# bytedance/DeepSolid

Hardware: AMD Instinct MI355X
Metric: local-energy evals/sec (higher is better)
Workload: dtype f64; 1 GPU; bcc_li 24 e- (12,12), total_energy primal (E_kin forward-Laplacian + Ewald), default detnet ((256,32),)*3, 8 dets; batch_per_gpu=4096, global_batch=4096, parallelism=walker-dp1

## Files before the change

### deepsolid_amd/_lib.py

```python
import ctypes as C
import os

_HERE = os.path.dirname(os.path.abspath(__file__))
LIB_PATH = os.environ.get('DEEPSOLID_HIP_LIB') or os.path.join(_HERE, 'libdeepsolid_hip.so')

DS_MAX_LAYERS = 8
DS_MAX_SYM = 6
_PD = C.POINTER(C.c_double)


class SystemDesc(C.Structure):
    _fields_ = [
        ('dtype', C.c_int32), ('n_up', C.c_int32), ('n_dn', C.c_int32), ('n_atoms_prim', C.c_int32),
        ('prim_atoms', _PD), ('prim_a', C.c_double * 9), ('sim_a', C.c_double * 9), ('n_sym', C.c_int32),
        ('prim_AV', C.c_double * (DS_MAX_SYM * 3)), ('prim_BV', C.c_double * (DS_MAX_SYM * 3)),
        ('sim_AV', C.c_double * (DS_MAX_SYM * 3)), ('sim_BV', C.c_double * (DS_MAX_SYM * 3)),
        ('n_layers', C.c_int32), ('hidden_single', C.c_int32 * DS_MAX_LAYERS),
        ('hidden_double', C.c_int32 * DS_MAX_LAYERS), ('n_det', C.c_int32), ('distance_type', C.c_int32),
        ('envelope_type', C.c_int32), ('full_det', C.c_int32), ('use_last_layer', C.c_int32),
        ('bias_orbitals', C.c_int32), ('klist_up', _PD), ('klist_dn', _PD),
        ('n_atoms_sim', C.c_int32), ('sim_atoms', _PD), ('sim_charges', _PD), ('dist_mode', C.c_int32),
        ('n_g', C.c_int32), ('gpoints', _PD), ('gweight', _PD), ('ion_exp_re', _PD), ('ion_exp_im', _PD),
        ('ewald_alpha', C.c_double), ('ee_const', C.c_double), ('ei_const', C.c_double), ('ii_total', C.c_double),
    ]


class ParamBlock(C.Structure):
    _fields_ = [('offset', C.c_int64), ('rows', C.c_int32), ('cols', C.c_int32)]


class KfacBlock(C.Structure):
    _fields_ = [('kind', C.c_int32), ('index', C.c_int32), ('n_param_blocks', C.c_int32), ('param_blocks', C.c_int32 * 3),
                ('has_bias', C.c_int32), ('d_in', C.c_int32), ('d_out', C.c_int32), ('repeats', C.c_int32),
                ('a_offset', C.c_int64), ('g_offset', C.c_int64)]


_VP = C.c_void_p
SIGNATURES = {
    'ds_device_widths': (C.c_int, [C.POINTER(C.c_int32), C.POINTER(C.c_int32), C.c_int32, C.c_int32, C.c_int32, C.c_int32,
                                   C.POINTER(C.c_int32), C.POINTER(C.c_int32), C.POINTER(C.c_int32), C.POINTER(C.c_int32)]),
    'ds_system_create': (C.c_int, [C.POINTER(SystemDesc), C.POINTER(_VP)]),
    'ds_system_destroy': (None, [_VP]),
    'ds_last_error': (C.c_char_p, []),
    'ds_param_count': (C.c_int64, [_VP]),
    'ds_int8_layers': (C.c_int, [_VP]),
    'ds_param_layout': (C.c_int, [_VP, C.POINTER(ParamBlock), C.c_int]),
    'ds_workspace_bytes': (C.c_int64, [_VP, C.c_int64]),
    'ds_logpsi': (C.c_int, [_VP, _VP, _VP, C.c_int64, _VP, _VP, _VP, C.c_int64, _VP]),
    'ds_logpsi_grad': (C.c_int, [_VP, _VP, _VP, C.c_int64, _VP, _VP, _VP, _VP, C.c_int64, _VP]),
    'ds_vjp_workspace_bytes': (C.c_int64, [_VP, C.c_int64]),
    'ds_logpsi_vjp': (C.c_int, [_VP, _VP, _VP, C.c_int64, _VP, _VP, _VP, _VP, _VP, C.c_int64, _VP]),
    'ds_pretrain_workspace_bytes': (C.c_int64, [_VP, C.c_int64]),
    'ds_pretrain_loss_vjp': (C.c_int, [_VP, _VP, _VP, C.c_int64, _VP, _VP, _VP, _VP, _VP, C.c_int64, _VP]),
    'ds_kfac_block_count': (C.c_int, [_VP]),
    'ds_kfac_layout': (C.c_int, [_VP, C.POINTER(KfacBlock), C.c_int]),
    'ds_kfac_workspace_bytes': (C.c_int64, [_VP, C.c_int64]),
    'ds_kfac_factors': (C.c_int, [_VP, _VP, _VP, C.c_int64, _VP, _VP, _VP, C.c_int64, _VP]),
    'ds_orbitals': (C.c_int, [_VP, _VP, _VP, C.c_int64, _VP, _VP, _VP, C.c_int64, _VP]),
    'ds_ewald': (C.c_int, [_VP, _VP, C.c_int64, _VP, _VP]),
    'ds_local_energy': (C.c_int, [_VP, _VP, _VP, C.c_int64, _VP, _VP, _VP, _VP, _VP, C.c_int64, _VP]),
    'ds_enforce_pbc': (C.c_int, [_PD, C.c_int, _VP, C.c_int64, _VP, _VP, _VP]),
    'ds_observables_workspace_bytes': (C.c_int64, [C.c_int64, C.c_int]),
    'ds_observables': (C.c_int, [_PD, C.c_int, _VP, C.c_int64, C.c_int64, C.POINTER(C.c_int32), C.c_int, C.c_int, _VP, _VP,
                                 C.c_int64, _VP]),
    'ds_mh_propose': (C.c_int, [_VP, _VP, _VP, C.c_double, C.c_int64, _VP, _VP]),
    'ds_mh_accept': (C.c_int, [_VP, _VP, _VP, _VP, _VP, _VP, C.c_int64, _VP, _VP]),
    'ds_mh_propose_ex': (C.c_int, [_VP, C.c_int, _VP, _VP, C.c_double, _VP, C.c_int, C.c_int64, _VP, _VP, _VP]),
    'ds_mh_accept_ex': (C.c_int, [_VP, C.c_int, _VP, _VP, _VP, _VP, _VP, _VP, C.c_double, _VP, _VP, C.c_int, C.c_int64, _VP, _VP, _VP]),
    'ds_mcmc_workspace_bytes': (C.c_int64, [_VP, C.c_int64]),
    'ds_mcmc_step': (C.c_int, [_VP, _VP, _VP, _VP, C.c_int64, C.c_int, C.c_double, C.c_uint64, C.c_uint64, _VP, _VP, C.c_int, _VP, _VP,
                              C.c_int64, _VP]),
    'ds_mcmc_step_one_electron': (C.c_int, [_VP, _VP, _VP, _VP, C.c_int64, C.c_int, C.c_int, C.c_double, C.c_uint64, C.c_uint64, _VP, _VP,
                                           C.c_int, _VP, _VP, C.c_int64, _VP]),
    'ds_mcmc_step_importance': (C.c_int, [_VP, _VP, _VP, _VP, C.c_int64, C.c_int, C.c_double, C.c_uint64, C.c_uint64, _VP, _VP, C.c_int,
                                         _VP, _VP, C.c_int64, _VP]),
    'ds_mcmc_step_asymmetric': (C.c_int, [_VP, _VP, _VP, _VP, C.c_int64, C.c_int, C.c_double, _VP, C.c_int, C.c_uint64, C.c_uint64, _VP, _VP,
                                         C.c_int, _VP, _VP, C.c_int64, _VP]),
    'ds_philox_host': (None, [C.c_uint64, C.c_uint64, C.c_uint64, C.c_uint64, C.c_int, C.POINTER(C.c_uint32)]),
# ... 38 lines not shown
```

### deepsolid_amd/csrc/ds_api.hip

```cpp
#include <hip/hip_runtime.h>

#include <algorithm>
#include <cmath>
#include <cstdarg>
#include <cstdio>
#include <cstdlib>
#include <cstring>
#include <string>
#include <vector>

#include "../../include/deepsolid_hip.h"
#include "ds_grad.h"
#include "ds_kfac.h"
#include "ds_tiles.h"
#include "ds_mcmc.h"
#include "ds_obs.h"
#include "ds_i8.h"

namespace ds {
#define DS_DECL(p) const TileOps<double>* tile_ops_f64_p##p(int); const TileOps<float>* tile_ops_f32_p##p(int);
DS_DECL(0) DS_DECL(1) DS_DECL(2) DS_DECL(3) DS_DECL(4)
#undef DS_DECL
template <> const TileOps<double>* tile_ops<double>(int st) {
    const TileOps<double>* (*parts[])(int) = {tile_ops_f64_p0, tile_ops_f64_p1, tile_ops_f64_p2, tile_ops_f64_p3, tile_ops_f64_p4};
// ... 359 lines not shown
    HIP_OK(hipMemcpyAsync(dr->out, src, m * sizeof(T), hipMemcpyDeviceToDevice, st));
    dr->written = (int64_t)m;
    return 0;
}

inline bool i8_shape(const ds_system* s, int l) {
    const ds::SysDev<double>& S = s->sd;
    return s->dtype == 0 && l >= 1 && s->res1[l] && S.h1[l + 1] == ds::i8::NOUT && S.h1[l] + S.nch * S.h2[l] == 320;
}
inline bool int8_value_layer(const ds_system* s, int l) { return s->use_i8_val && ds::PV == ds::i8::P && i8_shape(s, l); }

inline void i8_prepare(ds_system* s, int l, const double* Wloc, int Kloc, int Nout, hipStream_t st, uint8_t** wp, double** sw) {
    const size_t slot = ds::i8::wp_bytes(64 * 5) + ds::i8::NOUT * sizeof(double);
    *wp = (uint8_t*)s->i8_wp + (size_t)l * slot;
    *sw = (double*)(*wp + ds::i8::wp_bytes(64 * 5));
    if (s->i8_prepped[l] != s->call_seq) {
        hipLaunchKernelGGL(ds::i8::k_i8_prep_w, dim3(ds::i8::NOUT / 16), dim3(256), 0, st, Wloc, Kloc, Nout, *wp, *sw);
        s->i8_prepped[l] = s->call_seq;
    }
}

enum class LayerKind {
    Dense,
    DenseRes,
    L0Stats,
    L0Epi9Means,
    LowRank1,
    Int8
};
struct PairPlan {
    bool res, res_sep;
    bool expand;
    bool write_out;
    unsigned xz; int EW, NW; size_t xlds;
};
struct LayerPlan {
    LayerKind kind;
    bool res_sep;
    bool wide;
    bool pm_mask;
    bool pm_unwritten;
    int prof_kind;
    PairPlan pair;
};
enum class OrbKind { Orb3, Wide, Ldsb, Gemm };
template <typename T> struct ChainPlan {
    const ds::TileOps<T>* to;
    bool lr_on;
    int lr_nc;
    int g4;
    LayerPlan layer[DS_MAX_LAYERS];
    OrbKind orb[2];
    int count(LayerKind k, int n_layers) const {
        int n = 0;
        for (int l = 0; l < n_layers; ++l) n += layer[l].kind == k ? 1 : 0;
        return n;
    }
};

template <typename T>
int plan_chain(const ds_system* s, bool dump, ChainPlan<T>* p) {
    const ds::SysDev<double>& S = s->sd;
    const ds::TileOps<T>* to = p->to = ds::tile_ops<T>(S.P / 16);
    if (!to) return fail("no kernel instance for %d slot tiles (N = %d electrons)", S.P / 16, S.N);
    const int ST = to->ST;
    const bool wide = s->use_wide && to->gemm_wide != nullptr;
    auto gemm_wide = [&](int epi) { return wide && (s->wide_all || ds::gemm_wide_faster<T>(epi)); };
    const int K0loc = S.h1[0] + S.nch * S.h2[0], K0sh = S.nch * S.h1[0];
    p->lr_nc = std::max(2, (K0loc + K0sh + 4 + 15) / 16);
    p->lr_on = !dump && s->use_lr && S.n_layers >= 2 && !s->res1[0] && p->lr_nc <= 4 && S.h1[1] % 16 == 0 && (S.nch * S.h2[1]) % 4 == 0 &&
               3 * (K0loc + K0sh + 4) <= S.h1[1] && p->lr_nc * S.h1[1] < (S.h1[1] - K0loc - K0sh - 4) * ST;
    const int used = S.D - 16 * (ST - 1);
    p->g4 = !s->use_g4 ? 0 : (ST == 5 && used > 8 && used <= 12) ? 3 : (ST == 10 && used <= 4) ? 1 : 0;
    for (int l = 0; l < S.n_layers; ++l) {
        const int Kh = S.h1[l], K2 = S.h2[l], Nout = S.h1[l + 1], Kloc = Kh + S.nch * K2;
        LayerPlan& lp = p->layer[l];
        lp = LayerPlan{};
        if (Nout % 64 || Nout > 1024) return fail("hidden_single must be a multiple of 64 and <= 1024 (got %d)", Nout);
        if (l < S.n_double) {
            PairPlan& pp = lp.pair;
            const int K2o = S.h2[l + 1];
            if (K2o != 32 && K2o != 16) return fail("hidden_double must be 16 or 32 (got %d)", K2o);
            if (K2 % 4) return fail("pair-stream width %d is not a multiple of 4", K2);
            pp.res_sep = s->res2[l] && l == 0;
            pp.res = s->res2[l] && !pp.res_sep;
            pp.xz = (!pp.res && K2o == 32) ? 2 : 1;
            pp.write_out = l + 1 < S.n_double || s->use_last;
            pp.EW = (pp.write_out && S.N % 16 == 8 && pp.xz == 2) ? 2 : 1;
            pp.NW = (pp.EW * S.N + 15) / 16;
            pp.xlds = ((size_t)(K2o / pp.xz) * 5 * pp.EW * S.N + (size_t)pp.EW * S.nch * (K2o / pp.xz) * 5) * sizeof(T);
            pp.expand = !dump && s->use_pair_expand && !pp.res_sep && l + 1 < S.n_layers && pp.NW <= 8 && pp.xlds <= 150 * 1024;
        }
        const bool res = s->res1[l];
        lp.res_sep = res && l == 0 && (Kloc % 16 != 0 || S.nf * S.A != Nout);
        if (res && !lp.res_sep && Kloc % 16) return fail("residual layer with K = %d: the GEMM's operand ring needs K %% 16 == 0", Kloc);
        if (p->lr_on && l == 1) {
            lp.kind = LayerKind::LowRank1;
            lp.wide = wide && (s->wide_all || ds::lr_wide_faster<T>(p->lr_nc));
        } else if (p->lr_on && l == 0) {
            const bool one_kernel = to->layer0_stats && ds::layer0_stats_instance(ST, K0loc / 4);
            lp.kind = one_kernel ? LayerKind::L0Stats : LayerKind::L0Epi9Means;
            lp.wide = !one_kernel && gemm_wide(9);
        } else if (s->use_i8 && S.P == ds::i8::P && i8_shape(s, l)) {
            lp.kind = LayerKind::Int8;
        } else if (res && !lp.res_sep) {
            lp.kind = LayerKind::DenseRes;
            lp.wide = gemm_wide(2);
        } else {
            lp.kind = LayerKind::Dense;
            lp.wide = gemm_wide(1);
        }
        lp.prof_kind = l == 0 ? DS_PROF_SINGLE_FIRST : (lp.kind == LayerKind::LowRank1 ? DS_PROF_SINGLE_LR : DS_PROF_SINGLE_HIDDEN);
        lp.pm_mask = s->use_pm_skip && (l == 0 || (lp.kind == LayerKind::DenseRes && Kh % 16 == 0 && K2 % 16 == 0));
        lp.pm_unwritten = !dump && l >= 1 && !lp.wide &&
                          (lp.kind == LayerKind::LowRank1 ? s->use_pm_skip : (lp.pm_mask && ds::pm_instance<T>(ST)));
    }
    const int Korb = S.h1[S.n_layers] + (s->use_last ? S.nch * S.h2[S.n_layers] : 0);
    if (Korb % 16) return fail("orbital head with K = %d: the GEMM's operand ring needs K %% 16 == 0", Korb);
    for (int sp = 0; sp < S.nch; ++sp) {
        const int OC = S.ocols[sp];
        if (to->gemm_orb3 && OC % 256 != 0 && OC % 192 == 0) p->orb[sp] = OrbKind::Orb3;
        else if (gemm_wide(5)) p->orb[sp] = OrbKind::Wide;
        else if (to->orbital_lb && s->use_ldsb && OC % 64 == 0) p->orb[sp] = OrbKind::Ldsb;
        else p->orb[sp] = OrbKind::Gemm;
// ... 80 lines not shown
    const bool lr_on = plan.lr_on;
    const int K0loc = S.h1[0] + S.nch * S.h2[0], K0sh = S.nch * S.h1[0];
    {
        ProfScope ps(s, DS_PROF_FEATURES, st);
        size_t sh = (size_t)(9 * S.N) * sizeof(T) + (size_t)S.N * S.A * S.nf * sizeof(ds::Jet5<T>);
        hipLaunchKernelGGL((ds::k_features<T>), dim3((unsigned)Bc), dim3(256), sh, st, S, x, blk(s->i_pi[0]), blk(s->i_sg[0]),
                           blk(s->i_pi[S.nch - 1]), blk(s->i_sg[S.nch - 1]), lr_on ? c.XL : c.G[0], lr_on ? K0loc : S.ldk, c.MEAN[0], c.H2[0], c.Q);
    }
    if (lr_on) {
        const int n = S.h1[1] * 16 * lr_nc;
        hipLaunchKernelGGL((ds::k_lr_w0t<T>), dim3((unsigned)((n + 255) / 256)), dim3(256), 0, st, blk(s->i_wloc[0]), blk(s->i_wsh[0]), K0loc, K0sh,
                           S.h1[1], 16 * lr_nc, (T*)s->lr_w0t);
    }
    if (stop == STOP_MEAN0) return copy_out(dr, c.MEAN[0], (size_t)S.nch * S.h1[0] * S.P * Bc, st);
    if (stop == STOP_H2_0) return copy_out(dr, c.H2[0], (size_t)S.h2[0] * 5 * S.NP * Bc, st);
    if (stop == STOP_Q) return copy_out(dr, c.Q, L.Q * Bc, st);
    int gi = 0, hi = 0;
    for (int l = 0; l < S.n_layers; ++l) {
        const LayerPlan& lp = plan.layer[l];
        const int Kh = S.h1[l], K2 = S.h2[l], Nout = S.h1[l + 1];
        if (!(l > 0 && plan.layer[l - 1].pair.expand)) {
            ProfScope ps(s, DS_PROF_M2_EXPAND, st);
            const bool xl = lr_on && l == 0;
            hipLaunchKernelGGL((ds::k_m2_expand<T>), dim3(S.N, (unsigned)Bc, m2_split<T>(K2, S.N)), dim3(256), (size_t)(K2 * 5 * S.N + S.nch * K2 * 5) / m2_split<T>(K2, S.N) * sizeof(T), st, S,
                               c.H2[hi], K2, xl ? c.XL : c.G[gi], Kh, xl ? K0loc : S.ldk, lp.pm_unwritten ? 1 : 0);
        }
        if (stop == STOP_G0 + l) return copy_out(dr, c.G[gi], L.G * Bc, st);
        if (l < S.n_double) {
            const PairPlan& pp = lp.pair;
            const int K2o = S.h2[l + 1];
            const T* W2 = blk(s->i_w2[l]); const T* b2 = blk(s->i_b2[l]);
            ProfScope ps(s, DS_PROF_TWO_LAYER, st);
            if (pp.expand) {
#define DS_TWOX(NT2, RES) hipLaunchKernelGGL((ds::k_two_layer_expand<T, NT2, RES>), dim3(S.N / pp.EW, (unsigned)Bc, pp.xz), dim3(64 * pp.NW), pp.xlds, st, S, c.H2[hi], K2, W2, b2, \
                                             pp.write_out ? c.H2[hi ^ 1] : (T*)nullptr, c.G[gi ^ 1], S.h1[l + 1], S.ldk, plan.layer[l + 1].pm_unwritten ? 1 : 0, pp.EW)
                if (K2o == 32 && pp.res) DS_TWOX(2, true);
                else if (pp.res) DS_TWOX(1, true);
                else DS_TWOX(1, false);
#undef DS_TWOX
            } else {
                const dim3 grid((S.NP / 16 + 3) / 4, (unsigned)Bc);
#define DS_TWO(NT2, RES) hipLaunchKernelGGL((ds::k_two_layer<T, NT2, RES, false>), grid, dim3(256), 0, st, S, c.H2[hi], K2, W2, b2, c.H2[hi ^ 1])
                if (K2o == 32) { if (pp.res) DS_TWO(2, true); else DS_TWO(2, false); }
                else { if (pp.res) DS_TWO(1, true); else DS_TWO(1, false); }
#undef DS_TWO
            }
            if (pp.res_sep)
                hipLaunchKernelGGL((ds::k_pair_res_add<T>), dim3((unsigned)(((size_t)K2o * 5 * S.NP + 255) / 256), (unsigned)Bc), dim3(256), 0, st, c.H2[hi], K2, c.H2[hi ^ 1], K2o,
                                   S.nf, S.NP);
        }
        const int Kloc = Kh + S.nch * K2, Ksh = S.nch * Kh;
        {
            dim3 block; unsigned gz;
            gemm_geom(Nout, NB, &block, &gz, ST);
            dim3 wblock; unsigned wgz;
            gemm_geom(Nout, 4, &wblock, &wgz, 6);
            const size_t gws = (size_t)S.N * S.ldk * S.P, gts = (size_t)S.ldk * S.P;
            const bool lr1 = lp.kind == LayerKind::LowRank1;
            T* Sl = lr1 ? c.ZB + (size_t)Bc * S.h1[1] * S.P : c.ZB;
            {
                ProfScope ps(s, DS_PROF_SHARED_TERM, st);
                if (l == 0 || lr1) {
                    const ds::GemmArgs<T> ga{nullptr, 0, 0, nullptr, 0, l == 0 ? c.MEAN[0] : c.MEAN[1], (size_t)Ksh * S.P, blk(s->i_wsh[l]), Ksh, 0,
                                             Sl, (size_t)Nout * S.P, 0, Nout, S.P, nullptr, blk(s->i_b[l]), ds::OrbEpi<T>{}};
                    to->gemm(6, dim3(1, (unsigned)Bc, gz), block, st, ga);
                } else {
                    dim3 sblock; unsigned sgz;
                    gemm_geom(Nout, NB, &sblock, &sgz);
                    if (ST > 10 && sblock.x > 512) { sblock = dim3(512); sgz = (unsigned)((Nout / (16 * NB) + 7) / 8); }
                    to->shared_term(dim3(1, (unsigned)Bc, sgz), sblock, 2 * 16 * S.P * sizeof(T), st, S, c.G[gi], blk(s->i_wsh[l]), Kh, Sl, Nout, S.P,
                                    blk(s->i_b[l]), 0);
                }
// ... 23 lines not shown
            case LayerKind::L0Epi9Means: {
                ga.Z = c.YO; ga.zws = L.YO; ga.zts = (size_t)2 * Nout;
                layer_gemm(9, ga);
                constexpr int STC = 5;
                const unsigned nfb = (unsigned)((Nout + 63) / 64), nck = (unsigned)((S.P / 16 + STC - 1) / STC);
                hipLaunchKernelGGL((ds::k_layer0_means<T, STC>), dim3(S.nch * nfb * nck, (unsigned)Bc), dim3(256), 0, st, S, c.XL,
                                   (size_t)S.N * K0loc * S.P, (size_t)K0loc * S.P, blk(s->i_wloc[0]), K0loc, c.ZB, Nout, S.P, c.YO, c.MEAN[1]);
                break;
            }
            case LayerKind::Int8: {
                uint8_t* wp; double* sw;
                i8_prepare(s, l, (const double*)blk(s->i_wloc[l]), Kloc, Nout, st, &wp, &sw);
                const int ntiles = (int)(Bc * S.N);
                const dim3 igrid((unsigned)std::min<int64_t>(ntiles, s->n_cu));
                hipLaunchKernelGGL((ds::i8::k_layer_i8<5, 2>), igrid, dim3(512), ds::i8::lds_bytes(), st, (const double*)c.G[gi], gts, (const uint4*)wp,
                                   (const double*)sw, (const double*)Sl, S.N, (double*)c.G[gi ^ 1], ntiles);
                break;
            }
            case LayerKind::DenseRes:
                ga.oe.dbg = s->dbg & 3;
                ga.oe.g4 = plan.g4;
                if (l > 0 && s->prof_on && (s->prof_only < 0 || s->prof_only == DS_PROF_SINGLE_HIDDEN)) { ga.oe.clk = s->clk_dev; ga.oe.dbg = s->dbg; }
                layer_gemm(2, ga);
                break;
            case LayerKind::Dense:
                layer_gemm(1, ga);
                if (lp.res_sep)
                    hipLaunchKernelGGL((ds::k_layer_res_add<T>), dim3(S.N, (unsigned)Bc), dim3(256), 0, st, Xin, xws, xts, c.G[gi ^ 1], gws, gts, S.nf * S.A, Nout, S.P);
                break;
            }
        }
        gi ^= 1;
        if (l < S.n_double) {
            hi ^= 1;
            if (stop == STOP_H2_1 + l) return copy_out(dr, c.H2[hi], (size_t)S.h2[l + 1] * 5 * S.NP * Bc, st);
        }
    }
    if (stop == STOP_G0 + S.n_layers) return copy_out(dr, c.G[gi], L.G * Bc, st);
    const int Kl = S.h1[S.n_layers], K2l = S.h2[S.n_layers];
    if (s->use_last) {
        ProfScope ps(s, DS_PROF_M2_EXPAND, st);
        hipLaunchKernelGGL((ds::k_m2_expand<T>), dim3(S.N, (unsigned)Bc, m2_split<T>(K2l, S.N)), dim3(256), (size_t)(K2l * 5 * S.N + S.nch * K2l * 5) / m2_split<T>(K2l, S.N) * sizeof(T), st, S,
                           c.H2[hi], K2l, c.G[gi], Kl, S.ldk, 0);
    }
    for (int sp = 0; sp < S.nch; ++sp) {
        const int ns = sp == 0 ? S.n_up : S.n_dn, i0 = sp == 0 ? 0 : S.n_up, OC = S.ocols[sp];
        const int Korb = Kl + (s->use_last ? S.nch * K2l : 0);
        dim3 block; unsigned gz;
        gemm_geom(OC, NB, &block, &gz, ST);
        if (s->use_last) {
            ProfScope ps(s, DS_PROF_SHARED_TERM, st);
            to->shared_term(dim3(1, (unsigned)Bc, gz), block, 2 * 16 * S.P * sizeof(T), st, S, c.G[gi], blk(s->i_wsh_orb[sp]), Kl, c.ZB, OC, S.P,
                            (const T*)nullptr, 0);
        }
        ProfScope ps(s, DS_PROF_ORBITAL, st);
        const int ch = S.mat_ch[sp];
        ds::OrbEpi<T> oe{c.Q, c.MOUT, L.MOUT, L.mout_off[ch], S.N, i0, S.nparam[sp], S.nparam_max, S.norb[sp], S.det_n[ch],
                         S.row_off[sp], S.bias_orb ? blk(s->i_borb[sp]) : (const T*)nullptr, nullptr};
        oe.g4 = plan.g4;
        const ds::GemmArgs<T> ga{c.G[gi] + (size_t)i0 * S.ldk * S.P, (size_t)S.N * S.ldk * S.P, (size_t)S.ldk * S.P, blk(s->i_worb[sp]), Korb,
                                 nullptr, 0, nullptr, 0, ns, nullptr, 0, 0, OC, S.P, s->use_last ? (const T*)c.ZB : (const T*)nullptr, nullptr, oe};
        dim3 ob; unsigned oz;
        switch (plan.orb[sp]) {
        case OrbKind::Orb3:
            gemm_geom(OC, 3, &ob, &oz);
            to->gemm_orb3(dim3(ns * oz, (unsigned)Bc, 1), ob, st, ga);
            break;
// ... 1124 lines not shown
    s->wide_all = getenv("DS_WIDE_ALL") != nullptr;
    {
        ChainPlan<double> plan;
        bool need = plan_chain<double>(s, true, &plan) == 0 && plan.count(LayerKind::Int8, s->sd.n_layers) > 0;
        for (int l = 1; l < s->sd.n_layers; ++l) need = need || int8_value_layer(s, l);
        if (need && hipMalloc(&s->i8_wp, (size_t)DS_MAX_LAYERS * (ds::i8::wp_bytes(64 * 5) + ds::i8::NOUT * sizeof(double))) != hipSuccess) {
            ds_system_destroy(s);
            return fail("hipMalloc of the int8 layer's weight planes failed");
        }
    }
    if (const char* e = getenv("DS_CHUNK_WALKERS")) s->chunk_cap = std::min<int64_t>(65535, std::max<int64_t>(1, atol(e)));
    *out = s;
    return 0;
}

void ds_system_destroy(ds_system* s) {
    if (!s) return;
    if (s->clk_dev) (void)hipFree(s->clk_dev);
    if (s->lr_w0t) (void)hipFree(s->lr_w0t);
    if (s->i8_wp) (void)hipFree(s->i8_wp);
    if (s->blob64) (void)hipFree(s->blob64);
    if (s->blob32) (void)hipFree(s->blob32);
    delete s;
}

int64_t ds_param_count(const ds_system* s) { return s ? s->nparams : -1; }

int ds_int8_layers(const ds_system* s) {
    if (!s) return -1;
    ChainPlan<double> plan;
    return plan_chain<double>(s, false, &plan) == 0 ? plan.count(LayerKind::Int8, s->sd.n_layers) : 0;
}

int ds_param_layout(const ds_system* s, ds_param_block* blocks, int max_blocks) {
    if (!s) return -1;
    const int n = (int)s->blocks.size();
    for (int i = 0; i < n && i < max_blocks; ++i) blocks[i] = s->blocks[i];
    return n;
}

int64_t ds_workspace_bytes(const ds_system* s, int64_t B) {
    if (!s) return -1;
    const int64_t esz = s->dtype == 0 ? 8 : 4;
    int64_t budget = (int64_t)80 << 30;
    size_t free_b = 0, total_b = 0;
    if (hipMemGetInfo(&free_b, &total_b) == hipSuccess && free_b > 0)
        budget = std::min<int64_t>(budget, std::max<int64_t>((int64_t)(free_b / 10 * 4), (int64_t)1 << 30));
    const int64_t cap = s->chunk_cap;
    int64_t chunk = std::min<int64_t>(std::max<int64_t>(B, 1), cap);
    chunk = std::max<int64_t>(1, std::min<int64_t>(chunk, budget / ((int64_t)s->ws.per_walker * esz)));
    int64_t groups = std::min<int64_t>((std::max<int64_t>(B, 1) + ds::PV - 1) / ds::PV, 64);
    groups = std::max<int64_t>(1, std::min<int64_t>(groups, budget / ((int64_t)s->wsv.per_walker * esz)));
    return std::max((int64_t)s->ws.per_walker * esz * chunk, (int64_t)s->wsv.per_walker * esz * groups) + 256;
}

int ds_local_energy(ds_system* s, const void* params, const void* x, int64_t B, void* out_ke, void* out_ewald, void* out_logabs,
                    void* out_phase, void* ws, int64_t ws_bytes, void* stream) {
    if (s) ++s->call_seq;
    if (!s || !params || !x || !ws) return fail("null argument");
    if (B <= 0) return 0;
    hipStream_t st = (hipStream_t)stream;
    return s->dtype == 0 ? local_energy_impl<double>(s, params, x, B, out_ke, out_ewald, out_logabs, out_phase, ws, ws_bytes, st)
                         : local_energy_impl<float>(s, params, x, B, out_ke, out_ewald, out_logabs, out_phase, ws, ws_bytes, st);
}

int ds_logpsi(ds_system* s, const void* params, const void* x, int64_t B, void* out_logabs, void* out_phase, void* ws,
// ... 455 lines not shown
```

### deepsolid_amd/csrc/ds_kernels.h

```cpp
#pragma once
#include "ds_device.h"

namespace ds {

#define DS_MAXL 8

template <typename T> struct SysDev {
    int N, n_up, n_dn, A, L, K, nch;
    int D, P, NP;
    int n_layers, n_double;
    int h1[DS_MAXL + 1];
    int h2[DS_MAXL + 1];
    int ldk;
    int full_det, env_type, bias_orb;
    int dist_type, nf;
    int norb[2];
    int n_detch;
    int det_n[2];
    int mat_ch[2], row_off[2];
    int nparam[2];
    int nparam_max;
    int ocols[2];
    const T *prim_a, *prim_ainv, *sim_a, *sim_ainv, *prim_AV, *prim_BV, *sim_AV, *sim_BV, *atoms;
    const T* klist[2];
// ... 269 lines not shown
        pm_last = pm_valid && (lr == 15 || seg_of(p + 1) != sg);
    }
#pragma unroll
    for (int a = 0; a < NT2; ++a)
#pragma unroll
        for (int r = 0; r < 4; ++r) {
            const int n = 16 * a + acc_row<T>(lane, r);
            const T z0 = acc[a][0][r] + bias[n];
            const T y = ds_tanh(z0), d1 = 1 - y * y, d2 = -2 * y * d1;
            const T z1 = acc[a][1][r], z2 = acc[a][2][r], z3 = acc[a][3][r], z4 = acc[a][4][r];
            T o[5] = {y, d1 * z1, d1 * z2, d1 * z3, d1 * z4 + d2 * 2 * (z1 * z1 + z2 * z2 + z3 * z3)};
            if (VAL) {
                o[1] = ds_tanh(z1 + bias[n]); o[2] = ds_tanh(z2 + bias[n]); o[3] = ds_tanh(z3 + bias[n]); o[4] = ds_tanh(z4 + bias[n]);
            }
#pragma unroll
            for (int c = 0; c < 5; ++c) {
                T v = o[c];
                if (RES) v = ((KEEP ? bk[KEEP ? 4 * a + r : 0][c] : Hw[(size_t)(n * 5 + c) * NP]) + v) * rs2;
                if (Hout) Ho[(size_t)(n * 5 + c) * NP] = v;
                if (VAL && PARTM) {
                    const T pre = row16_prefix(pm_valid ? v : T(0));
                    if (pm_last) pm_lds[(pm_slot * Kout + n) * 5 + c] = pre;
                }
            }
        }
    if (VAL && PARTM) {
        __builtin_amdgcn_fence(__ATOMIC_ACQ_REL, "wavefront");
        __builtin_amdgcn_wave_barrier();
        T* pm = PARTM + ((size_t)w * (NP / 16) + pt) * (PM_SLOTS * Kout * 5);
        for (int i = lane; i < PM_SLOTS * Kout * 5; i += 64) pm[i] = pm_lds[i];
    }
}

template <typename T, int NT2, bool RES>
__global__ void __launch_bounds__(512) k_two_layer_expand(SysDev<T> S, const T* __restrict__ Hin, int Kin, const T* __restrict__ W,
                                                          const T* __restrict__ bias, T* __restrict__ Hout, T* __restrict__ G, int row0,
                                                          int ldg, int skip, int EW) {
    typedef typename Acc4<T>::type acc_t;
    extern __shared__ __attribute__((aligned(16))) char smem_raw[];
    const int w = blockIdx.y, wave = threadIdx.x >> 6, lane = threadIdx.x & 63, tid = threadIdx.x, nt = blockDim.x;
    const int N = S.N, NP = S.NP, P = S.P, Kout = 16 * NT2, e0 = blockIdx.x * EW, PW = EW * N;
    const int KT = Kout * gridDim.z, n0 = Kout * blockIdx.z;
    const int lr = lane & 15, lq = lane >> 4;
    const bool valid = wave * 16 + lr < PW;
    const int pl = valid ? wave * 16 + lr : PW - 1;
    const T* Hw = Hin + (size_t)w * Kin * 5 * NP + e0 * N + pl;
    T* hs = reinterpret_cast<T*>(smem_raw);
    T* sums = hs + Kout * 5 * PW;
    acc_t acc[NT2][5];
#pragma unroll
    for (int a = 0; a < NT2; ++a)
#pragma unroll
        for (int c = 0; c < 5; ++c) acc[a][c] = acc_t{0, 0, 0, 0};
    constexpr bool KEEP = RES && sizeof(T) == 8;
    T bk[KEEP ? 4 * NT2 : 1][5];
    if constexpr (KEEP) {
#pragma unroll
        for (int ks = 0; ks < 4 * NT2; ++ks)
#pragma unroll
            for (int c = 0; c < 5; ++c) bk[ks][c] = Hw[(size_t)((4 * ks + lq) * 5 + c) * NP];
#pragma unroll
        for (int ks = 0; ks < 4 * NT2; ++ks) {
            T av[NT2];
#pragma unroll
            for (int a = 0; a < NT2; ++a) av[a] = W[(size_t)(4 * ks + lq) * KT + n0 + 16 * a + lr];
#pragma unroll
            for (int a = 0; a < NT2; ++a)
#pragma unroll
                for (int c = 0; c < 5; ++c) acc[a][c] = mfma16(av[a], bk[ks][c], acc[a][c]);
        }
    } else
    for (int ks = 0; ks < Kin / 4; ++ks) {
        T av[NT2], bv[5];
#pragma unroll
        for (int a = 0; a < NT2; ++a) av[a] = W[(size_t)(4 * ks + lq) * KT + n0 + 16 * a + lr];
#pragma unroll
        for (int c = 0; c < 5; ++c) bv[c] = Hw[(size_t)((4 * ks + lq) * 5 + c) * NP];
#pragma unroll
        for (int a = 0; a < NT2; ++a)
#pragma unroll
            for (int c = 0; c < 5; ++c) acc[a][c] = mfma16(av[a], bv[c], acc[a][c]);
    }
    const T rs2 = T(0.70710678118654752440);
    T* Ho = (Hout && valid) ? Hout + ((size_t)w * KT + n0) * 5 * NP + e0 * N + pl : nullptr;
#pragma unroll
    for (int a = 0; a < NT2; ++a)
#pragma unroll
        for (int r = 0; r < 4; ++r) {
            const int n = 16 * a + acc_row<T>(lane, r);
            const T z0 = acc[a][0][r] + bias[n0 + n];
            const T y = ds_tanh(z0), d1 = 1 - y * y, d2 = -2 * y * d1;
            const T z1 = acc[a][1][r], z2 = acc[a][2][r], z3 = acc[a][3][r], z4 = acc[a][4][r];
            const T o[5] = {y, d1 * z1, d1 * z2, d1 * z3, d1 * z4 + d2 * 2 * (z1 * z1 + z2 * z2 + z3 * z3)};
// ... 1017 lines not shown
```

### deepsolid_amd/device.py

```python
import ctypes as C

import numpy as np
import torch

from . import _lib

_DTYPES = {torch.float64: 0, torch.float32: 1}


def _pd(a):
    return a.ctypes.data_as(C.POINTER(C.c_double))


def _ptr(t):
    return C.c_void_p(t.data_ptr()) if t is not None else C.c_void_p(0)


def _stream():
    return C.c_void_p(torch.cuda.current_stream().cuda_stream)


def _require_gpu():
    if not torch.cuda.is_available():
        raise RuntimeError('deepsolid_amd needs a ROCm GPU: there is no CPU path (the CPU oracle lives in '
# ... 551 lines not shown
                self._ws.numel(), _stream()), 'ds_mcmc_step_importance')
            return n_accept
        if first_electron is not None:
            _lib.check(self.lib.ds_mcmc_step_one_electron(
                self.handle, _ptr(p), _ptr(x), _ptr(lp), B, int(steps), int(first_electron), float(width), int(seed) & (2 ** 64 - 1),
                int(offset) & (2 ** 64 - 1), _ptr(normals), _ptr(uniforms), int(bool(lp_valid)), _ptr(n_accept), _ptr(self._ws),
                self._ws.numel(), _stream()), 'ds_mcmc_step_one_electron')
            return n_accept
        _lib.check(self.lib.ds_mcmc_step(self.handle, _ptr(p), _ptr(x), _ptr(lp), B, int(steps), float(width),
                                         int(seed) & (2 ** 64 - 1), int(offset) & (2 ** 64 - 1), _ptr(normals), _ptr(uniforms),
                                         int(bool(lp_valid)), _ptr(n_accept), _ptr(self._ws), self._ws.numel(), _stream()),
                   'ds_mcmc_step')
        return n_accept

    def energy_stats(self, ke, ew):
        out = torch.empty(8, dtype=torch.float64, device=self.device)
        _lib.check(self.lib.ds_energy_stats(self.handle, _ptr(ke), _ptr(ew), ke.shape[0], _ptr(out), _stream()), 'ds_energy_stats')
        return out

    def profile(self, on=True, only=None):
        mode = 0 if not on else (1 if only is None else 2 + _lib.PROF_KINDS.index(only))
        _lib.check(self.lib.ds_profile_enable(self.handle, mode), 'ds_profile_enable')

    def profile_read(self):
        n = len(_lib.PROF_KINDS)
        ms = (C.c_double * n)()
        cnt = (C.c_int64 * n)()
        _lib.check(self.lib.ds_profile_read(self.handle, ms, cnt), 'ds_profile_read')
        return {k: (float(ms[i]), int(cnt[i])) for i, k in enumerate(_lib.PROF_KINDS)}

    def int8_layers(self):
        return int(self.lib.ds_int8_layers(self.handle))

    def profile_clock(self):
        cyc, ticks = C.c_double(0), C.c_double(0)
        _lib.check(self.lib.ds_profile_read_clock(self.handle, C.byref(cyc), C.byref(ticks)), 'ds_profile_read_clock')
        return cyc.value, ticks.value, (cyc.value / ticks.value * 0.1 if ticks.value > 0 else None)

    def debug_stage(self, params, x, stage, n_elems):
        x = self._check_x(x)
        p = self.pack_params(params)
        ws = self.workspace(x.shape[0])
        out = torch.zeros(int(n_elems), dtype=self.dtype, device=self.device)
        n = self.lib.ds_debug_stage(self.handle, _ptr(p), _ptr(x), x.shape[0], stage.encode(), _ptr(out), out.numel(),
                                    _ptr(ws), ws.numel(), _stream())
        if n < 0:
            raise RuntimeError(f'ds_debug_stage({stage}): {self.lib.ds_last_error().decode()}')
        return out[:n]


def observable_sums(recvec, x, q_int, pol_direction):
    _require_gpu()
    if not x.is_cuda:
        raise RuntimeError('observable_sums: walkers must live on the ROCm device (no CPU path)')
    if x.dtype not in _DTYPES:
        raise TypeError(f'observable_sums: walkers must be float64 or float32, got {x.dtype}')
    if x.dim() != 2 or x.shape[1] % 3:
        raise ValueError(f'observable_sums: walkers must have shape (B, 3N), got {tuple(x.shape)}')
    if x.shape[0] < 1:
        raise ValueError('observable_sums: empty walker batch (the observables are batch means)')
    lib = _lib.load()
    x = x.contiguous()
    rv = np.ascontiguousarray(np.asarray(recvec, dtype=np.float64).reshape(3, 3))
    q = np.ascontiguousarray(np.asarray(q_int, dtype=np.int32).reshape(-1, 3))
    B, n_q = x.shape[0], q.shape[0]
    need = lib.ds_observables_workspace_bytes(B, n_q)
# ... 7 lines not shown
```

### include/deepsolid_hip.h

```cpp
#ifndef DEEPSOLID_HIP_H
#define DEEPSOLID_HIP_H

#include <stddef.h>
#include <stdint.h>

#ifdef __cplusplus
extern "C" {
#endif

#define DS_MAX_LAYERS 8
#define DS_MAX_SYM 6

typedef struct ds_system ds_system;

typedef struct ds_system_desc {
    int32_t dtype;
    int32_t n_up, n_dn;
    int32_t n_atoms_prim;
    const double* prim_atoms;
    double prim_a[9];
    double sim_a[9];
    int32_t n_sym;
    double prim_AV[DS_MAX_SYM * 3], prim_BV[DS_MAX_SYM * 3];
    double sim_AV[DS_MAX_SYM * 3], sim_BV[DS_MAX_SYM * 3];
// ... 7 lines not shown
    int32_t use_last_layer;
    int32_t bias_orbitals;
    const double* klist_up;
    const double* klist_dn;
    int32_t n_atoms_sim;
    const double* sim_atoms;
    const double* sim_charges;
    int32_t dist_mode;
    int32_t n_g;
    const double* gpoints;
    const double* gweight;
    const double* ion_exp_re;
    const double* ion_exp_im;
    double ewald_alpha;
    double ee_const;
    double ei_const;
    double ii_total;
} ds_system_desc;

typedef struct ds_param_block {
    int64_t offset;
    int32_t rows, cols;
} ds_param_block;

int ds_device_widths(const int32_t* hidden_single, const int32_t* hidden_double, int32_t n_layers, int32_t n_in_single,
                     int32_t n_in_double, int32_t n_double, int32_t* dev_single, int32_t* dev_double, int32_t* res_single,
                     int32_t* res_double);

int ds_system_create(const ds_system_desc* desc, ds_system** out);
void ds_system_destroy(ds_system* sys);
const char* ds_last_error(void);

int ds_int8_layers(const ds_system* sys);

int64_t ds_param_count(const ds_system* sys);
int ds_param_layout(const ds_system* sys, ds_param_block* blocks, int max_blocks);

int64_t ds_workspace_bytes(const ds_system* sys, int64_t B);

int ds_logpsi(ds_system* sys, const void* params, const void* x, int64_t B,
              void* out_logabs, void* out_phase, void* ws, int64_t ws_bytes, void* stream);

int ds_logpsi_grad(ds_system* sys, const void* params, const void* x, int64_t B,
                   void* out_logabs, void* out_phase, void* out_grad, void* ws, int64_t ws_bytes, void* stream);

int64_t ds_vjp_workspace_bytes(const ds_system* sys, int64_t B);
int ds_logpsi_vjp(ds_system* sys, const void* params, const void* x, int64_t B, const void* cot, void* grad,
                  void* out_logabs, void* out_phase, void* ws, int64_t ws_bytes, void* stream);

int64_t ds_pretrain_workspace_bytes(const ds_system* sys, int64_t B);
int ds_pretrain_loss_vjp(ds_system* sys, const void* params, const void* x, int64_t B, const void* target_up,
                         const void* target_dn, void* out_loss, void* grad, void* ws, int64_t ws_bytes, void* stream);

typedef struct ds_kfac_block {
    int32_t kind, index;
    int32_t n_param_blocks;
    int32_t param_blocks[3];
    int32_t has_bias, d_in, d_out, repeats;
    int64_t a_offset, g_offset;
} ds_kfac_block;
int ds_kfac_block_count(const ds_system* sys);
int ds_kfac_layout(const ds_system* sys, ds_kfac_block* blocks, int max_blocks);
int64_t ds_kfac_workspace_bytes(const ds_system* sys, int64_t B);
int ds_kfac_factors(ds_system* sys, const void* params, const void* x, int64_t B, void* factors, void* grad_seed, void* ws,
                    int64_t ws_bytes, void* stream);

// ... 75 lines not shown
```

Baseline: 68540 local-energy evals/s.

## Recompute pair layer 0 inside fused layer-1 kernel instead of storing it

```diff
diff --git a/deepsolid_amd/_lib.py b/deepsolid_amd/_lib.py
--- a/deepsolid_amd/_lib.py
+++ b/deepsolid_amd/_lib.py
@@ -44,6 +44,7 @@
     'ds_last_error': (C.c_char_p, []),
     'ds_param_count': (C.c_int64, [_VP]),
     'ds_int8_layers': (C.c_int, [_VP]),
+    'ds_pair_recompute_layers': (C.c_int, [_VP]),
     'ds_param_layout': (C.c_int, [_VP, C.POINTER(ParamBlock), C.c_int]),
     'ds_workspace_bytes': (C.c_int64, [_VP, C.c_int64]),
     'ds_logpsi': (C.c_int, [_VP, _VP, _VP, C.c_int64, _VP, _VP, _VP, C.c_int64, _VP]),
diff --git a/deepsolid_amd/csrc/ds_api.hip b/deepsolid_amd/csrc/ds_api.hip
--- a/deepsolid_amd/csrc/ds_api.hip
+++ b/deepsolid_amd/csrc/ds_api.hip
@@ -415,6 +415,7 @@
     bool res, res_sep;
     bool expand;
     bool write_out;
+    bool recompute_prev;
     unsigned xz; int EW, NW; size_t xlds;
 };
 struct LayerPlan {
@@ -455,6 +456,13 @@
                3 * (K0loc + K0sh + 4) <= S.h1[1] && p->lr_nc * S.h1[1] < (S.h1[1] - K0loc - K0sh - 4) * ST;
     const int used = S.D - 16 * (ST - 1);
     p->g4 = !s->use_g4 ? 0 : (ST == 5 && used > 8 && used <= 12) ? 3 : (ST == 10 && used <= 4) ? 1 : 0;
+    auto pair_expand_fits = [&](int K2o, int xz) {
+        const size_t xlds = ((size_t)(K2o / xz) * 5 * S.N + (size_t)S.nch * (K2o / xz) * 5) * sizeof(T);
+        return (S.N + 15) / 16 <= 8 && xlds <= 150 * 1024;
+    };
+    const bool recompute1 = sizeof(T) == 8 && !dump && s->use_pair_expand && S.n_double >= 2 && S.n_layers >= 3 && !s->res2[0] && s->res2[1] &&
+                            S.h2[0] % 4 == 0 && S.h2[1] == S.h2[2] && (S.h2[1] == 16 || S.h2[1] == 32) &&
+                            pair_expand_fits(S.h2[1], S.h2[1] == 32 ? 2 : 1) && pair_expand_fits(S.h2[2], 1);
     for (int l = 0; l < S.n_layers; ++l) {
         const int Kh = S.h1[l], K2 = S.h2[l], Nout = S.h1[l + 1], Kloc = Kh + S.nch * K2;
         LayerPlan& lp = p->layer[l];
@@ -468,11 +476,14 @@
             pp.res_sep = s->res2[l] && l == 0;
             pp.res = s->res2[l] && !pp.res_sep;
             pp.xz = (!pp.res && K2o == 32) ? 2 : 1;
-            pp.write_out = l + 1 < S.n_double || s->use_last;
+            pp.recompute_prev = recompute1 && l == 1;
+            pp.write_out = (l + 1 < S.n_double || s->use_last) && !(recompute1 && l == 0);
             pp.EW = (pp.write_out && S.N % 16 == 8 && pp.xz == 2) ? 2 : 1;
             pp.NW = (pp.EW * S.N + 15) / 16;
             pp.xlds = ((size_t)(K2o / pp.xz) * 5 * pp.EW * S.N + (size_t)pp.EW * S.nch * (K2o / pp.xz) * 5) * sizeof(T);
             pp.expand = !dump && s->use_pair_expand && !pp.res_sep && l + 1 < S.n_layers && pp.NW <= 8 && pp.xlds <= 150 * 1024;
+            if (pp.recompute_prev && !(pp.expand && pp.res && p->layer[0].pair.expand && !p->layer[0].pair.res && !p->layer[0].pair.res_sep))
+                return fail("pair layer 1 was planned to recompute layer 0, but the two layers do not run fused");
         }
         const bool res = s->res1[l];
         lp.res_sep = res && l == 0 && (Kloc % 16 != 0 || S.nf * S.A != Nout);
@@ -619,12 +630,19 @@
             const T* W2 = blk(s->i_w2[l]); const T* b2 = blk(s->i_b2[l]);
             ProfScope ps(s, DS_PROF_TWO_LAYER, st);
             if (pp.expand) {
+                T* const Hout = !pp.write_out ? (T*)nullptr : pp.recompute_prev ? c.H2[hi] : c.H2[hi ^ 1];
 #define DS_TWOX(NT2, RES) hipLaunchKernelGGL((ds::k_two_layer_expand<T, NT2, RES>), dim3(S.N / pp.EW, (unsigned)Bc, pp.xz), dim3(64 * pp.NW), pp.xlds, st, S, c.H2[hi], K2, W2, b2, \
-                                             pp.write_out ? c.H2[hi ^ 1] : (T*)nullptr, c.G[gi ^ 1], S.h1[l + 1], S.ldk, plan.layer[l + 1].pm_unwritten ? 1 : 0, pp.EW)
-                if (K2o == 32 && pp.res) DS_TWOX(2, true);
+                                             Hout, c.G[gi ^ 1], S.h1[l + 1], S.ldk, plan.layer[l + 1].pm_unwritten ? 1 : 0, pp.EW)
+#define DS_TWOXP(NT2) hipLaunchKernelGGL((ds::k_two_layer_expand<T, NT2, true, true>), dim3(S.N / pp.EW, (unsigned)Bc, pp.xz), dim3(64 * pp.NW), pp.xlds, st, S, c.H2[hi], K2, W2, b2, \
+                                         Hout, c.G[gi ^ 1], S.h1[l + 1], S.ldk, plan.layer[l + 1].pm_unwritten ? 1 : 0, pp.EW, c.H2[hi ^ 1], S.h2[0], blk(s->i_w2[0]), blk(s->i_b2[0]))
+                if (pp.recompute_prev) {
+                    if constexpr (sizeof(T) == 8) { if (K2o == 32) DS_TWOXP(2); else DS_TWOXP(1); }
+                }
+                else if (K2o == 32 && pp.res) DS_TWOX(2, true);
                 else if (pp.res) DS_TWOX(1, true);
                 else DS_TWOX(1, false);
 #undef DS_TWOX
+#undef DS_TWOXP
             } else {
                 const dim3 grid((S.NP / 16 + 3) / 4, (unsigned)Bc);
 #define DS_TWO(NT2, RES) hipLaunchKernelGGL((ds::k_two_layer<T, NT2, RES, false>), grid, dim3(256), 0, st, S, c.H2[hi], K2, W2, b2, c.H2[hi ^ 1])
@@ -714,7 +732,7 @@
         }
         gi ^= 1;
         if (l < S.n_double) {
-            hi ^= 1;
+            if (!lp.pair.recompute_prev) hi ^= 1;
             if (stop == STOP_H2_1 + l) return copy_out(dr, c.H2[hi], (size_t)S.h2[l + 1] * 5 * S.NP * Bc, st);
         }
     }
@@ -1905,6 +1923,17 @@
     return plan_chain<double>(s, false, &plan) == 0 ? plan.count(LayerKind::Int8, s->sd.n_layers) : 0;
 }
 
+int ds_pair_recompute_layers(const ds_system* s) {
+    if (!s) return -1;
+    auto count = [&](auto plan) {
+        int n = 0;
+        if (plan_chain(s, false, &plan) != 0) return 0;
+        for (int l = 0; l < s->sd.n_double; ++l) n += plan.layer[l].pair.recompute_prev ? 1 : 0;
+        return n;
+    };
+    return s->dtype == 0 ? count(ChainPlan<double>{}) : count(ChainPlan<float>{});
+}
+
 int ds_param_layout(const ds_system* s, ds_param_block* blocks, int max_blocks) {
     if (!s) return -1;
     const int n = (int)s->blocks.size();
diff --git a/deepsolid_amd/csrc/ds_kernels.h b/deepsolid_amd/csrc/ds_kernels.h
--- a/deepsolid_amd/csrc/ds_kernels.h
+++ b/deepsolid_amd/csrc/ds_kernels.h
@@ -325,10 +325,12 @@
     }
 }
 
-template <typename T, int NT2, bool RES>
+template <typename T, int NT2, bool RES, bool PRE = false>
 __global__ void __launch_bounds__(512) k_two_layer_expand(SysDev<T> S, const T* __restrict__ Hin, int Kin, const T* __restrict__ W,
                                                           const T* __restrict__ bias, T* __restrict__ Hout, T* __restrict__ G, int row0,
-                                                          int ldg, int skip, int EW) {
+                                                          int ldg, int skip, int EW, const T* __restrict__ H0 = nullptr, int Kin0 = 0,
+                                                          const T* __restrict__ W0 = nullptr, const T* __restrict__ bias0 = nullptr) {
+    static_assert(!PRE || (RES && sizeof(T) == 8), "PRE: the remade input lands in the kept operands of a float64 residual layer");
     typedef typename Acc4<T>::type acc_t;
     extern __shared__ __attribute__((aligned(16))) char smem_raw[];
     const int w = blockIdx.y, wave = threadIdx.x >> 6, lane = threadIdx.x & 63, tid = threadIdx.x, nt = blockDim.x;
@@ -348,10 +350,37 @@
     constexpr bool KEEP = RES && sizeof(T) == 8;
     T bk[KEEP ? 4 * NT2 : 1][5];
     if constexpr (KEEP) {
+        if constexpr (PRE) {
+            const T* H0w = H0 + (size_t)w * Kin0 * 5 * NP + e0 * N + pl;
+            for (int ks = 0; ks < Kin0 / 4; ++ks) {
+                T av[NT2], bv[5];
+#pragma unroll
+                for (int a = 0; a < NT2; ++a) av[a] = W0[(size_t)(4 * ks + lq) * Kout + 16 * a + lr];
+#pragma unroll
+                for (int c = 0; c < 5; ++c) bv[c] = H0w[(size_t)((4 * ks + lq) * 5 + c) * NP];
+#pragma unroll
+                for (int a = 0; a < NT2; ++a)
+#pragma unroll
+                    for (int c = 0; c < 5; ++c) acc[a][c] = mfma16(av[a], bv[c], acc[a][c]);
+            }
+#pragma unroll
+            for (int a = 0; a < NT2; ++a)
+#pragma unroll
+                for (int r = 0; r < 4; ++r) {
+                    const int n = 16 * a + acc_row<T>(lane, r);
+                    const T z0 = acc[a][0][r] + bias0[n];
+                    const T y = ds_tanh(z0), d1 = 1 - y * y, d2 = -2 * y * d1;
+                    const T z1 = acc[a][1][r], z2 = acc[a][2][r], z3 = acc[a][3][r], z4 = acc[a][4][r];
+                    const T o[5] = {y, d1 * z1, d1 * z2, d1 * z3, d1 * z4 + d2 * 2 * (z1 * z1 + z2 * z2 + z3 * z3)};
+#pragma unroll
+                    for (int c = 0; c < 5; ++c) { bk[KEEP ? 4 * a + r : 0][c] = o[c]; acc[a][c][r] = 0; }
+                }
+        } else {
 #pragma unroll
         for (int ks = 0; ks < 4 * NT2; ++ks)
 #pragma unroll
             for (int c = 0; c < 5; ++c) bk[ks][c] = Hw[(size_t)((4 * ks + lq) * 5 + c) * NP];
+        }
 #pragma unroll
         for (int ks = 0; ks < 4 * NT2; ++ks) {
             T av[NT2];
diff --git a/deepsolid_amd/device.py b/deepsolid_amd/device.py
--- a/deepsolid_amd/device.py
+++ b/deepsolid_amd/device.py
@@ -607,6 +607,9 @@
     def int8_layers(self):
         return int(self.lib.ds_int8_layers(self.handle))
 
+    def pair_recompute_layers(self):
+        return int(self.lib.ds_pair_recompute_layers(self.handle))
+
     def profile_clock(self):
         cyc, ticks = C.c_double(0), C.c_double(0)
         _lib.check(self.lib.ds_profile_read_clock(self.handle, C.byref(cyc), C.byref(ticks)), 'ds_profile_read_clock')
diff --git a/include/deepsolid_hip.h b/include/deepsolid_hip.h
--- a/include/deepsolid_hip.h
+++ b/include/deepsolid_hip.h
@@ -63,6 +63,8 @@
 const char* ds_last_error(void);
 
 int ds_int8_layers(const ds_system* sys);
+
+int ds_pair_recompute_layers(const ds_system* sys);
 
 int64_t ds_param_count(const ds_system* sys);
 int ds_param_layout(const ds_system* sys, ds_param_block* blocks, int max_blocks);
```

Result: no change. 68890 local-energy evals/s (median of 6 runs) (+0.5%).
